# CasperTheCat/Vermilion

Measured on AMD Instinct MI355X. Metric: Mrays/sec (primary+secondary), 1920x1080 Sponza, higher is better.
Workload: dtype f32

## Files before the change

### vermilion_amd/csrc/api_render.inc

```
namespace {

Tuning make_tuning(const vmx_scene *sc, const vmx_opts *o) {
    Tuning tn;
    tn.refill_min = o->reserved[3] ? o->reserved[3] : 8u;
    tn.refill_primary = o->reserved[3] ? o->reserved[3] : 64u;
    tn.shade_min = o->reserved[4] ? o->reserved[4] : 16u;
    tn.leaf_min = 0xFFFFFFFFu;
    tn.sort_mode = o->reserved[5];
    tn.two_phase = false;
    tn.sorted = false;
    tn.bounce_records = false;
    tn.pool = false;
    tn.guide = false;
    const uint32_t cap = o->reserved[6];
    tn.lds_entries = std::min(sc->dev.stack_entries, cap ? cap : 10u);
    tn.lds_primary = std::min(sc->dev.stack_entries, cap ? cap : (uint32_t)VMX_LDS_PRIMARY);
    tn.lds_bounce = std::min(sc->dev.stack_entries, cap ? cap : 9u);
    tn.tail_threshold = o->reserved[2] ? o->reserved[2] : (16u << 20);
    return tn;
}


int bind_stack(vmx_scene *sc, const Tuning &tn, uint32_t entries, uint32_t grid, uint64_t items, WorkDev &wk, bool guided = false) {
    const uint64_t per_lane = items / ((uint64_t)grid * kPathsBlock);
// ... 368 lines not shown
        if (ws.full_mask.ensure(words + 8) || ws.full_u32.ensure(2 * words + 16) || ws.full_tmp.ensure(tmp + 256))
            return fail(VMX_ERR_NOMEM, "hipMalloc failed for the two-phase shading lists");
        ws.full_words = words, ws.full_tmp_bytes = tmp;
    }
    if (job.split_any && (tn.sorted || tn.bounce_records)) {
        const size_t waves = (size_t)sc->num_cus * ((size_t)std::max(job.tb, job.tbb) + (tn.guide ? kGuideFallbackBlocks : 0u)) * (kPathsBlock / 64);
        ws.out_capacity = (size_t)n_pad_max * smax + waves * 256 + 1024;
        if (ws.out_capacity > 0xFFFFFFFFull) return fail(VMX_ERR_INVALID, "pass too large for the sorted ray records");
        if (ws.out_rec.ensure(ws.out_capacity * (tn.sorted ? 32 : 16)) || ws.out_count.ensure(32))
            return fail(VMX_ERR_NOMEM, "hipMalloc failed for the ray records");
    }
    if (job.split_any) {
        if (ws.guide_ctr.ensure(2) || (tn.guide && (ws.guide_fb.ensure((size_t)job.qi[0].sub_capacity * kSubQueues) ||
                                                    ws.guide_fb_count.ensure(32) || ws.guide_heads.ensure(32))))
            return fail(VMX_ERR_NOMEM, "hipMalloc failed for the guide tree's fallback list");
    }
    if (job.elide) {
        if (ws.live_mask.ensure(job.live_words_max + 8) || ws.live_u32.ensure(2 * job.live_words_max + 16) ||
            ws.live_ids.ensure((size_t)n_pad_max * smax + 64) || ws.live_tmp.ensure(job.live_tmp_bytes + 256))
            return fail(VMX_ERR_NOMEM, "hipMalloc failed for the live-path list");
    }
    if (ws.rad.ensure((size_t)n_pad_max * smax * 16) || ws.next_count.ensure(32) || ws.counters.ensure(1) ||
        (tn.guide && ws.guide_fused_ctr.ensure(2)))
        return fail(VMX_ERR_NOMEM, "hipMalloc failed for the render workspace");
    job.px = PixelStateDev{job.pixels->accum.p, job.pixels->count.p, job.pixels->cursor.p};
    if (job.split_any) {
        const size_t n_inner = std::max<size_t>(sc->n_inner, 1);
        if (ws.cam_inner.ensure(n_inner * 64 * 8 + (size_t)sc->ntris * 64))
            return fail(VMX_ERR_NOMEM, "hipMalloc failed for the camera tables");
        LAUNCH_TRY(launch_camera_tables(sc->dev, sc->n_inner, fr.px, fr.py, fr.pz, ws.cam_inner.p,
                                        ws.cam_inner.p + n_inner * 64 * 8, s));
        job.launches++;
    }
    job.claims = job.claim_lists = nullptr;
    if (job.claims_on) {
        uint32_t expect = fr.early_stop ? std::min(fr.kmax, fr.nmin + 1 + (fr.quarter ? fr.kmax / fr.quarter - 1u : 0u)) : fr.kmax;
        if (run_samples) expect = std::min(expect, run_samples);
        if (expect >= claim_min_samples()) {
            int rc = timed_begin(ws, job.timed, s, -1, VMX_K_OTHER);
            if (rc) return rc;
            if ((rc = build_claims(sc, fr, tn, job.npix, job.lists_on, s))) return rc;
            if ((rc = timed_end(job.timed, s))) return rc;
            job.claims = ws.claims.p;
            if (job.lists_on) job.claim_lists = ws.claim_lists.p;
            job.launches++;
        }
    }
    if (job.claims && job.fuse_on) {
        const size_t words = n_pad_max / 64;
        const size_t tmp = live_compact_tmp_bytes((uint32_t)words);
        if (ws.unclaimed.ensure((size_t)n_pad_max + 64) || ws.claimed_slots.ensure((size_t)n_pad_max + 64) || ws.unclaimed_mask.ensure(words + 8) || ws.unclaimed_u32.ensure(2 * words + 16) ||
            ws.unclaimed_tmp.ensure(tmp + 256))
            return fail(VMX_ERR_NOMEM, "hipMalloc failed for the list of unclaimed pixels");
        ws.unclaimed_words = words, ws.unclaimed_tmp_bytes = tmp;
    }
    return VMX_OK;
}

int render_pass(vmx_scene *sc, RenderJob &job, uint32_t cap, uint32_t *taken) {
    Workspace &ws = sc->ws;
    FrameDev &fr = job.fr;
    const Tuning &tn = job.tn;
    const uint32_t pipeline = job.pipeline, smax = job.smax, n_active = job.n_active, n_pad_max = job.n_pad_max;
    const bool count = job.count, elide = job.elide;
    const int cur_list = job.cur_list;
    PixelStateDev px = job.px;
    PathArrays &pa = job.pa;
    IdQueue *qi = job.qi;
    hipStream_t s = job.s;
    std::vector<TimedLaunch> &timed = job.timed;
    uint64_t &launches = job.launches;
    unsigned int *act_cur = job.pixels->active[cur_list].p, *act_next = job.pixels->active[cur_list ^ 1].p;
    int rc;
    *taken = 0;
    uint32_t S;
    if (fr.early_stop) {
        fr.lead = 0;
        if (job.n_uniform < fr.nmin + 1 && job.n_uniform < fr.kmax) {
            S = std::min({fr.nmin + 1 - job.n_uniform, smax, fr.kmax - job.n_uniform, cap});
            job.n_uniform += S;
            const uint32_t strata_after = fr.quarter ? fr.kmax / fr.quarter - 1u : 0u;
            if (S == fr.nmin + 1 && S <= fr.quarter && strata_after > 0 && S + strata_after <= std::min(smax, cap)) {
                fr.lead = S;
                S += strata_after;
            }
        } else {
            constexpr uint64_t spec = 16ull << 20, spec_cap = 1024;
            S = std::max(1u, fr.kmax / std::max(fr.quarter, 1u) - 1u);
            if ((job.last_pass_pixels > 0 && job.last_pass_breaks * 8 < job.last_pass_pixels) || (uint64_t)n_active * 2 * spec_cap <= spec)
                S = (uint32_t)std::min<uint64_t>(std::max<uint64_t>(1, spec / (2ull * n_active)), spec_cap);
            S = (uint32_t)std::min<uint64_t>(S, ((uint64_t)n_pad_max * job.smax_alloc) / ((n_active + 63u) & ~63u));
            S = std::max(std::min(S, cap), 1u);
        }
    } else if (job.ragged) {
        S = std::min(smax, cap);
    } else {
        if (job.k_fixed >= fr.kmax) {
            job.n_active = 0;
            return VMX_OK;
        }
        S = std::min({smax, fr.kmax - job.k_fixed, cap});
        job.k_fixed += S;
    }
    *taken = S;
    const uint32_t n_pad = (n_active + 63u) & ~63u;
    const bool split = pipeline == 4 || (pipeline == 0 && (uint64_t)n_pad * S >= ((fr.early_stop && job.frame_passes > 0) ? kHybridLeftover : kHybridPaths));
    const bool refill = pipeline == 1 || (pipeline == 0 && !split);
    WorkDev wk;
    std::memset(&wk, 0, sizeof(wk));
    wk.heads = ws.heads.p;
    wk.nsrc = 8;
    wk.refill_min = split ? tn.refill_primary : tn.refill_min, wk.shade_min = tn.shade_min;
    wk.active = act_cur;
    wk.n_active = n_active, wk.n_pad = n_pad, wk.samples = S, wk.div_samples = make_fastdiv(S);
    wk.band_slots = (((n_pad + 7u) / 8u) + 63u) & ~63u;
    wk.band_items = wk.band_slots * S;
    wk.pixel_major = 1;
    if (split) {
        wk.cam_inner = ws.cam_inner.p, wk.cam_tris = ws.cam_inner.p + std::max<size_t>(sc->n_inner, 1) * 64 * 8;
        wk.cam_n_inner = sc->n_inner;
        wk.claims = job.claims;
        wk.claim_lists = elide ? nullptr : job.claim_lists, wk.list_ctr = ws.counters.p;
        const bool fuse = job.fuse_on && job.claims && (S & 63u) == 0;
        LaunchCfg cfg = paths_cfg(sc, tn.lds_primary, (uint64_t)n_pad * S, job.tb);
        rc = bind_stack(sc, tn, tn.lds_primary, cfg.grid, (uint64_t)n_pad * S, wk);
        if (rc) return rc;
        HIP_TRY(hipMemsetAsync(ws.heads.p, 0, kSubQueues * 32 * 4, s));
        if ((rc = timed_begin(ws, timed, s, -1, VMX_K_RAYGEN))) return rc;
        if (elide) {
            const uint32_t nwords = (uint32_t)(((uint64_t)n_pad * S + 63) / 64);
            unsigned int *cnt = ws.live_u32.p, *offs = cnt + job.live_words_max, *len = offs + job.live_words_max;
            wk.live_mask = ws.live_mask.p, wk.live_cnt = cnt;
            LAUNCH_TRY(launch_raygen(sc->dev, fr, wk, px, pa, s));
            HIP_TRY((hipError_t)launch_live_compact(ws.live_mask.p, cnt, nwords, offs, ws.live_ids.p, len, ws.live_tmp.p, job.live_tmp_bytes, s));
            wk.live_ids = ws.live_ids.p, wk.live_count = len;
            LAUNCH_TRY(launch_raygen_live(sc->dev, fr, wk, px, pa, s));
            HIP_TRY(hipMemsetAsync(pa.rad_mask, 0, (size_t)nwords * 8, s));
        } else {
            if (fuse) {
                const uint32_t nwords = n_pad / 64;
                unsigned int *cnt = ws.unclaimed_u32.p, *offs = cnt + ws.unclaimed_words, *len = offs + ws.unclaimed_words;
                LAUNCH_TRY(launch_unclaimed_words(act_cur, n_active, n_pad, job.claims, ws.unclaimed_mask.p, cnt, s));
                HIP_TRY((hipError_t)launch_slot_lists(ws.unclaimed_mask.p, cnt, nwords, n_active, offs, ws.unclaimed.p, ws.claimed_slots.p, len,
                                                      ws.unclaimed_tmp.p, ws.unclaimed_tmp_bytes, s));
                wk.unclaimed = ws.unclaimed.p, wk.unclaimed_count = len;
                launches += 3;
            }
            LAUNCH_TRY(launch_raygen(sc->dev, fr, wk, px, pa, s));
        }
        if (tn.sorted) {
            wk.out_rec = ws.out_rec.p, wk.out_count = ws.out_count.p, wk.out_ctr = ws.counters.p, wk.out_capacity = (uint32_t)ws.out_capacity;
            HIP_TRY(hipMemsetAsync(ws.out_count.p, 0, 4, s));
            if (!elide) HIP_TRY(hipMemsetAsync(pa.rad_mask, 0, (size_t)(((uint64_t)n_pad * S + 63) / 64) * 8, s));
        }
        if ((rc = timed_end(timed, s))) return rc;
        if ((rc = timed_begin(ws, timed, s, 0, VMX_K_TRACE_CAMERA))) return rc;
        {
            WorkDev wt = wk;
            if (fuse) wt.claims = nullptr;
            LAUNCH_TRY(launch_trace_q(sc->dev, fr, wt, px, pa, ws.counters.p, count, false, cfg, s));
        }
        if ((rc = timed_end(timed, s))) return rc;
        HIP_TRY(hipMemsetAsync(qi[0].counts, 0, kSubQueues * 32 * 4, s));
        if ((rc = timed_begin(ws, timed, s, 2, VMX_K_SHADE_CAMERA))) return rc;
        if (tn.two_phase && !elide && !tn.sorted) {
            if ((rc = shade_two_phase(sc, fr, wk, px, pa, qi, qi[0], 0, (size_t)(((uint64_t)n_pad * S + 63) / 64), false, ws.counters.p, false, s))) return rc;
        } else {
            if (fuse) {
                WorkDev wsh = wk;
                wsh.shade_slots = wk.unclaimed, wsh.shade_count = wk.unclaimed_count;
                LAUNCH_TRY(launch_shade(sc->dev, fr, wsh, px, pa, qi[0], 0, ws.counters.p, false, s));
                wsh.shade_slots = ws.claimed_slots.p, wsh.shade_count = wk.unclaimed_count + 1, wsh.fused = 1;
                LAUNCH_TRY(launch_shade(sc->dev, fr, wsh, px, pa, qi[0], 0, ws.counters.p, false, s));
                launches++;
            } else {
                LAUNCH_TRY(launch_shade(sc->dev, fr, wk, px, pa, qi[0], 0, ws.counters.p, false, s));
            }
        }
        if ((rc = timed_end(timed, s))) return rc;
        launches += 4;
        rc = run_ids(sc, fr, pa, qi, 0, ws.counters.p, count, tn, s, timed, launches, job.tbb, job.rb);
        if (rc) return rc;
    } else if (refill) {
        LaunchCfg cfg = paths_cfg(sc, tn.lds_entries, (uint64_t)n_pad * S, job.rb);
        rc = bind_stack(sc, tn, tn.lds_entries, cfg.grid, (uint64_t)n_pad * S, wk, tn.guide);
        if (rc) return rc;
        HIP_TRY(hipMemsetAsync(ws.heads.p, 0, kSubQueues * 32 * 4, s));
        if ((rc = timed_begin(ws, timed, s, 0, VMX_K_FUSED))) return rc;
        const GuidePathsDev gp = guide_paths(sc, tn);
        LAUNCH_TRY(launch_paths(sc->dev, fr, wk, px, ws.rad.p, ws.counters.p, count, cfg, s, &gp));
        if ((rc = timed_end(timed, s))) return rc;
        launches += 2;
    } else {
        rc = ab_legacy_pass(sc, job, act_cur, n_active, S);
        if (rc) return rc;
    }
    HIP_TRY(hipMemsetAsync(ws.next_count.p, 0, 8, s));
    if ((rc = timed_begin(ws, timed, s, -1, VMX_K_RESOLVE))) return rc;
    LAUNCH_TRY(launch_resolve(fr, act_cur, n_active, S, split || refill, ws.rad.p, split ? pa.rad_mask : nullptr, px, act_next,
                              ws.next_count.p, job.d_out, ws.counters.p, s, job.moments));
    if ((rc = timed_end(timed, s))) return rc;
    launches++;
    job.passes++;
    job.frame_passes++;
    unsigned int h_next[2] = {0, 0};
    HIP_TRY(hipMemcpyAsync(h_next, ws.next_count.p, 8, hipMemcpyDeviceToHost, s));
    HIP_TRY(hipStreamSynchronize(s));
    job.last_pass_pixels = n_active;
    job.last_pass_breaks = h_next[1];
    job.n_active = h_next[0];
    job.cur_list ^= 1;
    return VMX_OK;
// ... 436 lines not shown
```

### vermilion_amd/csrc/vmx_host.h

```cpp
namespace {

thread_local std::string g_err;

int fail(int code, const std::string &msg) {
    g_err = msg;
    return code;
}

#define HIP_TRY(expr)                                                                              \
    do {                                                                                           \
        hipError_t e_ = (expr);                                                                    \
        if (e_ != hipSuccess)                                                                      \
            return fail(VMX_ERR_HIP, std::string(#expr) + ": " + hipGetErrorString(e_));           \
    } while (0)

#define LAUNCH_TRY(expr)                                                                           \
    do {                                                                                           \
        int e_ = (expr);                                                                           \
        if (e_ != 0)                                                                               \
            return fail(VMX_ERR_HIP, std::string(#expr) + ": " + hipGetErrorString((hipError_t)e_)); \
    } while (0)

const vmx_sphere kReferenceSpheres[8] = {
    {{15.f, 140.f, 25.f}, 3.5f, {0.f * 15.f, .5f * 15.f, 1.0f * 15.f}, VMX_SPHERE_EMIT, {-55.f, 350.f, -150.f}, -1.f},
// ... 60 lines not shown
            hipEvent_t e;
            if (hipEventCreate(&e) != hipSuccess) return nullptr;
            ev.push_back(e);
        }
        return ev[used++];
    }
    void reset() { used = 0; }
};

struct Fence : NoCopy {
    hipEvent_t ev = nullptr;
    bool recorded = false;
    ~Fence() { if (ev) (void)hipEventDestroy(ev); }
    int wait(hipStream_t s) const {
        if (recorded) HIP_TRY(hipStreamWaitEvent(s, ev, 0));
        return VMX_OK;
    }
    int record(hipStream_t s) {
        if (!ev) HIP_TRY(hipEventCreateWithFlags(&ev, hipEventDisableTiming));
        HIP_TRY(hipEventRecord(ev, s));
        recorded = true;
        return VMX_OK;
    }
    int sync() const {
        if (recorded) HIP_TRY(hipEventSynchronize(ev));
        return VMX_OK;
    }
};

struct PixelBufs {
    DevBuf<unsigned char> accum;
    DevBuf<unsigned int> count, cursor, active[2];
    int ensure(size_t npix) {
        return accum.ensure(npix * 16) || count.ensure(npix) || cursor.ensure(npix) || active[0].ensure(npix) || active[1].ensure(npix);
    }
};

struct Workspace {
    DevBuf<unsigned char> queue_planes[2];
    DevBuf<unsigned int> queue_counts;
    DevBuf<unsigned int> heads;
    DevBuf<unsigned char> overflow_stack;
    DevBuf<unsigned char> rayA, state, hit, thr;
    DevBuf<unsigned int> ids[3], id_counts;
    DevBuf<unsigned int> sort_keys[2], ids_sorted;
    DevBuf<unsigned char> sort_tmp;
    DevBuf<unsigned char> cam_inner;
    DevBuf<unsigned int> claims;
    DevBuf<unsigned int> claim_lists;
    DevBuf<unsigned int> unclaimed, claimed_slots, unclaimed_u32;
    DevBuf<unsigned long long> unclaimed_mask;
    DevBuf<unsigned char> unclaimed_tmp;
    size_t unclaimed_words = 0, unclaimed_tmp_bytes = 0;
    DevBuf<unsigned char> rad;
    DevBuf<unsigned long long> rad_mask;
    DevBuf<unsigned long long> live_mask;
    DevBuf<unsigned int> live_u32, live_ids;
    DevBuf<unsigned char> live_tmp;
    DevBuf<unsigned long long> full_mask;
    DevBuf<unsigned int> full_u32;
    DevBuf<unsigned char> full_tmp;
    size_t full_words = 0, full_tmp_bytes = 0;
    DevBuf<unsigned char> out_rec;
    DevBuf<unsigned int> out_count;
    size_t out_capacity = 0;
    DevBuf<unsigned int> guide_fb, guide_fb_count, guide_heads;
    DevBuf<unsigned long long> guide_ctr;
    DevBuf<unsigned long long> guide_fused_ctr;
    uint64_t guide_entries = 0;
    PixelBufs pixels;
    DevBuf<unsigned int> next_count;
    DevBuf<DevCounters> counters;
    DevBuf<float> out;
    std::vector<unsigned int> order;
    uint32_t order_w = 0, order_rows = 0;
    EventPool events;
};

}

#define VMX_OPAQUE __attribute__((visibility("hidden")))

struct vmx_scene {
    int device = 0;
    int num_cus = 0;
    DevStream stream;
    HostBvh bvh;
    LbvhDevice lbvh;
    bool device_built = false;
    uint32_t builder = VMX_BVH_REFERENCE;
    std::atomic<bool> flat_ready{true};
    bool flat_topology = true;
    uint32_t n_inner = 0;
    uint32_t ntris = 0, leaf_size = 4;
    std::vector<vmx_sphere> spheres;
    DevBuf<unsigned char> d_geom;
    DevBuf<AttrRecord> d_attrs;
    DevBuf<SphereDev> d_spheres;
    DevBuf<float> d_tex, d_tex1;
    uint32_t n_textures = 0;
    SceneDev dev{};
    std::mutex mu;
    Workspace ws;
    uint32_t block = 256;
    float bounds_lo[3] = {0, 0, 0}, bounds_hi[3] = {1, 1, 1};
    vmx_timings timings{};
// ... 236 lines not shown
```

### vermilion_amd/csrc/vmx_kernels.h

```cpp
#pragma once
#include <stdint.h>
#include "vmx_device.h"

namespace vmx {

constexpr uint32_t kSubQueues = 16;

struct QueueDev {
    void *planes;
    unsigned int *counts;
    uint32_t capacity;
    uint32_t sub_capacity;
};

struct PixelStateDev {
    void *accum;
    unsigned int *count;
    unsigned int *cursor;
};

struct PathArrays {
    void *rayA;
    void *state;
    void *hit;
// ... 98 lines not shown
                   LaunchCfg cfg, void *stream);
int launch_primary_ids(const SceneDev &sc, const FrameDev &fr, uint32_t k, int32_t *tri_id, float *t,
                       LaunchCfg cfg, void *stream);

constexpr uint32_t kQueryCastRays = 3, kQueryCastCamera = 4, kQueryModes = 5;
int launch_query(const SceneDev &sc, const QueryDev &q, uint32_t mode, bool quad, LaunchCfg cfg, void *stream);
int query_query_blocks_per_cu(uint32_t block, uint32_t lds_bytes, uint32_t mode, bool quad, int *blocks);
int launch_raycast_query(const SceneDev &sc, const QueryDev &q, const FrameDev &fr, bool camera, bool quad, void *out,
                         LaunchCfg cfg, uint32_t finish_grid, void *stream);

struct RefitItem {
    uint32_t ref, dst;
};
constexpr uint32_t kRefitRoot = 0xFFFFFFFFu;
int launch_update_records(uint32_t ntris, const float *pos, const float *nrm, const float *uv, void *tris, void *attrs,
                          void *stream);
int launch_refit_level(const RefitItem *items, uint32_t n, const float *pos, const void *tris, void *inner,
                       float *root_box, void *stream);
int launch_attrs_by_id(uint32_t ntris, const void *tris, const void *attrs, float *nrm, float *uv, void *stream);

int launch_trig(const float *x, uint32_t n, float *cs, float *sn, void *stream);

int launch_init_pixels(PixelStateDev px, uint32_t npix, void *stream);
int launch_zero_u32(unsigned int *p, uint32_t n, void *stream);
#ifdef VMX_AB_KERNELS
int launch_primary(const SceneDev &sc, const FrameDev &fr, const unsigned int *active,
                   uint32_t n_active, uint32_t samples, PixelStateDev px, QueueDev qout, void *rad,
                   DevCounters *counters, bool count, bool loop_to_end, LaunchCfg cfg, void *stream);
int launch_radiance_init(const float *o, const float *d, uint32_t n, uint64_t seed, QueueDev qout,
                         void *stream);
int launch_bounce(const SceneDev &sc, float r2scale, uint32_t libm_double, QueueDev qin, uint32_t max_chunks, QueueDev qout,
                  void *rad, DevCounters *counters, bool count, bool loop_to_end, bool first_step,
                  LaunchCfg cfg, void *stream);
int query_blocks_per_cu(uint32_t block, uint32_t lds_bytes, bool count, int *primary_blocks, int *bounce_blocks);
int launch_trace_pool(const SceneDev &sc, const WorkDev &wk, PathArrays pa, LaunchCfg cfg, void *stream);
int query_trace_pool(uint32_t block, uint32_t pool_slots, uint32_t lds_levels, uint32_t *lds_bytes, int *blocks);
#endif
int launch_paths(const SceneDev &sc, const FrameDev &fr, const WorkDev &wk, PixelStateDev px, void *rad,
                 DevCounters *counters, bool count, LaunchCfg cfg, void *stream, const GuidePathsDev *guide = nullptr);
int query_paths_blocks_per_cu(uint32_t block, uint32_t lds_bytes, bool count, int *blocks, bool guide = false);
int launch_camera_tables(const SceneDev &sc, uint32_t n_inner, float ox, float oy, float oz, void *cam_inner,
                         void *cam_tris, void *stream);
int launch_pixel_claims(const SceneDev &sc, const FrameDev &fr, const WorkDev &wk, unsigned int *claims, unsigned int *lists, unsigned int *n_claimed,
                        LaunchCfg cfg, void *stream);
int launch_raygen(const SceneDev &sc, const FrameDev &fr, const WorkDev &wk, PixelStateDev px, PathArrays pa, void *stream);
int launch_raygen_live(const SceneDev &sc, const FrameDev &fr, const WorkDev &wk, PixelStateDev px, PathArrays pa, void *stream);
size_t live_compact_tmp_bytes(uint32_t nwords);
int launch_live_compact(const unsigned long long *live_mask, const unsigned int *live_cnt, uint32_t nwords,
                        unsigned int *offs, unsigned int *ids, unsigned int *count, void *tmp, size_t tmp_bytes, void *stream);
int launch_slot_lists(const unsigned long long *mask, const unsigned int *cnt, uint32_t nwords, uint32_t n_active, unsigned int *offs,
                      unsigned int *unclaimed, unsigned int *claimed, unsigned int *counts, void *tmp, size_t tmp_bytes, void *stream);
int launch_unclaimed_words(const unsigned int *active, uint32_t n_active, uint32_t n_pad, const unsigned int *claims,
                           unsigned long long *mask, unsigned int *cnt, void *stream);
int launch_trace_q(const SceneDev &sc, const FrameDev &fr, const WorkDev &wk, PixelStateDev px, PathArrays pa,
                   DevCounters *counters, bool count, bool from_queue, LaunchCfg cfg, void *stream, const GuideDev *guide = nullptr,
                   unsigned int *visits = nullptr);
int query_trace_q_blocks_per_cu(uint32_t block, uint32_t lds_bytes, bool count, bool from_queue, bool sorted, bool live, int *blocks,
                                bool guide = false);
int launch_shade(const SceneDev &sc, const FrameDev &fr, const WorkDev &wk, PixelStateDev px, PathArrays pa,
                 IdQueue qout, uint32_t max_chunks, DevCounters *counters, bool from_queue, void *stream);
int launch_shade_ends(const SceneDev &sc, const FrameDev &fr, const WorkDev &wk, PathArrays pa, unsigned long long *full_mask,
                      unsigned int *full_cnt, uint32_t max_chunks, DevCounters *counters, bool from_queue, void *stream);
int launch_tail(const SceneDev &sc, const FrameDev &fr, const WorkDev &wk, PathArrays pa, DevCounters *counters,
                bool count, LaunchCfg cfg, void *stream, const GuidePathsDev *guide = nullptr);
int launch_radiance_init_ids(const float *o, const float *d, uint32_t n, uint64_t seed, PathArrays pa,
                             IdQueue qout, void *stream);
int launch_resolve(const FrameDev &fr, const unsigned int *active, uint32_t n_active, uint32_t samples,
                   bool pixel_major, const void *rad, const unsigned long long *rad_mask, PixelStateDev px, unsigned int *next_active,
                   unsigned int *next_count, float *out_rgbaz, DevCounters *counters, void *stream, bool moments = false);
int launch_list_words(const unsigned int *list, uint32_t n, const unsigned char *select, const unsigned int *cursor, uint32_t kmax,
                      unsigned long long *mask, unsigned int *cnt, void *stream);
int launch_list_compact(const unsigned long long *mask, const unsigned int *cnt, uint32_t nwords, unsigned int *offs,
                        const unsigned int *src, unsigned int *dst, unsigned int *count, void *tmp, size_t tmp_bytes, void *stream);
struct SamplingPass {
    uint32_t width, height;
    uint32_t kmax, min_samples, radius;
    float threshold, floor;
    PixelStateDev px;
};
int launch_sampling_error(const SamplingPass &a, float *error, float *variance, void *stream);
int launch_sampling_select(const SamplingPass &a, unsigned char *select, unsigned int *count, void *stream);
int launch_bruteforce(const SceneDev &sc, const FrameDev &fr, const unsigned int *order, uint32_t npix, uint32_t flags,
                      float *out, DevCounters *counters, void *longs , unsigned int *long_count,
                      const WorkDev &stack , LaunchCfg cfg, void *stream);
int launch_bruteforce_long(const SceneDev &sc, const FrameDev &fr, uint32_t flags, float *out, DevCounters *counters,
                           const void *longs, const unsigned int *long_count, uint32_t count, const WorkDev &stack,
                           LaunchCfg cfg, void *stream);
int launch_preview(PixelStateDev px, uint32_t npix, uint32_t kmax, const float *finished, float *out_rgbaz, void *rgba8,
                   void *stream);
struct FilterSrc {
    const float *frame;
    PixelStateDev px;
    const float *finished;
    uint32_t kmax;
};
struct FilterPass {
    uint32_t width, height;
    uint32_t step;
    uint32_t squarings;
    float isc2, kz;
    const void *guide;
    FilterSrc src;
    const void *in_plane;
    void *out_plane;
    float *out_rgbaz;
    void *rgba8;
// ... 91 lines not shown
```

### vermilion_amd/csrc/vmx_kernels.hip

```cpp
#include <hip/hip_runtime.h>
#include <math.h>
#include <algorithm>
#include <stdint.h>

#include "vmx_kernels.h"
#include "pixel_claim.h"
#include "guide_walk.h"
#include <type_traits>

#ifndef VMX_CAM_BATCH
#define VMX_CAM_BATCH 16
#endif
#ifndef VMX_TRACE_WAVES_PER_SIMD
#define VMX_TRACE_WAVES_PER_SIMD 7
#endif


namespace vmx {
__device__ __forceinline__ float luminance(float r, float g, float b);
namespace {

constexpr float kInf = __builtin_huge_valf();

struct Cnt {
// ... 1446 lines not shown
    __device__ __forceinline__ void put(int i, uint32_t ref, float near) { stack_push(stk, ovf, lds_entries, i, make_uint2(ref, __float_as_uint(near))); }
    __device__ __forceinline__ void get(int i, uint32_t &ref, float &near) const {
        const uint2 e = stack_pop(stk, ovf, lds_entries, i);
        ref = e.x, near = __uint_as_float(e.y);
    }
};
__global__ void __launch_bounds__(256)
k_pixel_claims(SceneDev sc, FrameDev fr, const float *__restrict__ cam_inner, const float *__restrict__ cam_tris,
               unsigned int *__restrict__ claims, unsigned int *__restrict__ lists, unsigned int *n_claimed, uint32_t lds_levels,
               uint32_t overflow_entries, void *overflow_stack) {
    extern __shared__ uint2 lds_stack[];
    const uint32_t lane = threadIdx.x & 63u, wave = threadIdx.x >> 6;
    ClaimStack stk;
    stk.stk = lds_stack + (size_t)wave * (lds_levels + 1) * 64 + lane;
    stk.ovf = (uint2 *)overflow_stack + ((size_t)(blockIdx.x * (blockDim.x >> 6) + wave) * overflow_entries) * 64 + lane;
    stk.lds_entries = (int)lds_levels;
    PcFilm fm;
    for (int i = 0; i < 9; ++i) fm.m[i] = fr.m[i];
    fm.width = fr.width, fm.height = fr.height, fm.sensor_x = fr.sensor_x, fm.sensor_y = fr.sensor_y, fm.film_dist = fr.film_dist;
    const uint32_t tiles_x = (fr.width + 7u) / 8u, tiles = tiles_x * ((fr.local_rows + 7u) / 8u);
    uint32_t n = 0;
    for (uint32_t tile = blockIdx.x * (blockDim.x >> 6) + wave; tile < tiles; tile += gridDim.x * (blockDim.x >> 6)) {
        const uint32_t ty = tile / tiles_x, tx = tile - ty * tiles_x;
        const uint32_t x = tx * 8u + (lane & 7u), y = ty * 8u + (lane >> 3);
        if (x < fr.width && y < fr.local_rows) {
            const uint32_t lp = y * fr.width + x;
            uint32_t c;
            if (lists) {
                uint32_t l[kListWords];
                c = pc_pixel_claim_and_list(fm, global_pixel(fr, lp), cam_inner, cam_tris, sc.root_ref, stk,
                                            (int)(lds_levels + overflow_entries), l);
                ((uint4 *)lists)[lp] = make_uint4(l[0], l[1], l[2], l[3]);
            } else {
                c = pc_pixel_claim(fm, global_pixel(fr, lp), cam_inner, cam_tris, sc.root_ref, stk, (int)(lds_levels + overflow_entries));
            }
            claims[lp] = c;
            n += c != kClaimNone ? 1u : 0u;
        }
    }
    n = wave_sum(n);
    if (lane == 0 && n) atomicAdd(n_claimed, n);
}

__global__ void __launch_bounds__(256)
k_unclaimed_words(const unsigned int *__restrict__ active, uint32_t n_active, uint32_t n_pad, const unsigned int *__restrict__ claims,
                  unsigned long long *__restrict__ mask, unsigned int *__restrict__ cnt) {
    for (uint32_t s_idx = blockIdx.x * blockDim.x + threadIdx.x; s_idx < n_pad; s_idx += gridDim.x * blockDim.x) {
        const bool un = s_idx < n_active && claims[active[s_idx]] == kClaimNone;
        const unsigned long long bits = __builtin_amdgcn_ballot_w64(un);
        if ((threadIdx.x & 63u) == 0) mask[s_idx >> 6] = bits, cnt[s_idx >> 6] = (uint32_t)__popcll(bits);
    }
}

template <int LIVE>
__global__ void __launch_bounds__(256)
k_raygen(SceneDev sc, FrameDev fr, WorkDev wk, PixelStateDev px, PathArrays pa) {
    const uint32_t total = wk.samples * wk.n_pad;
    if (wk.pixel_major && (wk.samples & 63u) == 0) {
        const uint32_t lane = threadIdx.x & 63u;
        const uint32_t waves = gridDim.x * (blockDim.x >> 6);
        const uint32_t chunks = wk.samples >> 6;
        const bool listed = !LIVE && wk.unclaimed != nullptr;
        const uint32_t units = listed ? *wk.unclaimed_count : wk.n_pad;
        for (uint32_t unit = (uint32_t)__builtin_amdgcn_readfirstlane((int)(blockIdx.x * (blockDim.x >> 6) + (threadIdx.x >> 6)));
             unit < units; unit += waves) {
            const uint32_t s_idx = listed ? wk.unclaimed[unit] : unit;
            const uint32_t pid_base = s_idx * wk.samples;
            if (s_idx < wk.n_active) {
                const uint32_t lp = wk.active[s_idx];
                const uint32_t pixel = global_pixel(fr, lp);
                const PixelKey pk = rng_pixel_key(fr.seed, pixel);
                const bool lights = (LIVE || fr.camera_bits) && pixel_may_reach_a_light(sc, fr, pixel);
                const uint32_t cur = px.cursor[lp];
                const uint32_t k0 = cur & ~kCursorStrided, kstep = (cur & kCursorStrided) ? fr.quarter : 1u;
                for (uint32_t ch = 0; ch < chunks; ++ch) {
                    const uint32_t j = ch * 64u + lane;
                    const uint32_t k = (fr.lead != 0 && j >= fr.lead) ? (j - fr.lead + 1u) * fr.quarter : k0 + j * kstep;
                    bool live = false;
                    float dx = 0.f, dy = 0.f, dz = 0.f;
                    uint32_t depth = 0xFFFFFFFFu;
                    if (k < fr.kmax) {
                        Rng rng;
                        if (LIVE && !lights) {
                            rng_init_keyed(rng, pk, k);
                            (void)rng_next(rng);
                            (void)rng_next(rng);
                            live = step_bits<false>(sc, fr.r2scale, rng, 0, fr.px, fr.py, fr.pz, 0.f, 0.f, 0.f, 1.f, 1.f, 1.f, false) != 3u;
                        } else {
                            primary_ray_keyed(fr, pixel, pk, k, rng, dx, dy, dz);
                            if (LIVE) live = !step_is_dead<false>(sc, fr.r2scale, rng, 0, fr.px, fr.py, fr.pz, dx, dy, dz, 1.f, 1.f, 1.f);
                            else depth = fr.camera_bits ? step_bits<false>(sc, fr.r2scale, rng, 0, fr.px, fr.py, fr.pz, dx, dy, dz, 1.f, 1.f, 1.f, lights) : 0u;
                        }
                    }
                    if (!LIVE) ((float4 *)pa.rayA)[pid_base + j] = make_float4(dx, dy, dz, __uint_as_float(depth));
                    if (LIVE) {
                        const unsigned long long bits = __builtin_amdgcn_ballot_w64(live);
                        if (lane == 0) wk.live_mask[(pid_base >> 6) + ch] = bits, wk.live_cnt[(pid_base >> 6) + ch] = (uint32_t)__popcll(bits);
                    }
                }
            } else {
                for (uint32_t ch = 0; ch < chunks; ++ch) {
                    if (!LIVE) ((float4 *)pa.rayA)[pid_base + ch * 64u + lane] = make_float4(0.f, 0.f, 0.f, __uint_as_float(0xFFFFFFFFu));
                    if (LIVE && lane == 0) wk.live_mask[(pid_base >> 6) + ch] = 0ull, wk.live_cnt[(pid_base >> 6) + ch] = 0u;
                }
            }
        }
        return;
    }
    for (uint32_t pid = blockIdx.x * blockDim.x + threadIdx.x; pid < total; pid += gridDim.x * blockDim.x) {
        uint32_t j, s_idx;
        if (wk.pixel_major) s_idx = fast_div(pid, wk.div_samples), j = pid - s_idx * wk.samples;
        else j = pid / wk.n_pad, s_idx = pid - j * wk.n_pad;
        uint32_t pid2, pixel, k;
        float dx = 0.f, dy = 0.f, dz = 0.f;
        uint32_t depth = 0xFFFFFFFFu;
        bool live = false;
        if (s_idx < wk.n_active && primary_item(fr, wk, px, j, s_idx, pid2, pixel, k)) {
            Rng rng;
            primary_ray(fr, pixel, k, rng, dx, dy, dz);
            if (LIVE) live = !step_is_dead<false>(sc, fr.r2scale, rng, 0, fr.px, fr.py, fr.pz, dx, dy, dz, 1.f, 1.f, 1.f);
            else depth = fr.camera_bits ? step_bits<false>(sc, fr.r2scale, rng, 0, fr.px, fr.py, fr.pz, dx, dy, dz, 1.f, 1.f, 1.f) : 0u;
        }
        if (!LIVE) ((float4 *)pa.rayA)[pid] = make_float4(dx, dy, dz, __uint_as_float(depth));
        if (LIVE) {
            const unsigned long long bits = __builtin_amdgcn_ballot_w64(live);
            if ((threadIdx.x & 63u) == 0) wk.live_mask[pid >> 6] = bits, wk.live_cnt[pid >> 6] = (uint32_t)__popcll(bits);
        }
    }
}

__global__ void __launch_bounds__(256)
k_raygen_live(SceneDev sc, FrameDev fr, WorkDev wk, PixelStateDev px, PathArrays pa) {
    const uint32_t n = *wk.live_count;
    for (uint32_t i = blockIdx.x * blockDim.x + threadIdx.x; i < n; i += gridDim.x * blockDim.x) {
        const uint32_t pid = wk.live_ids[i];
        uint32_t j, s_idx;
        if (wk.pixel_major) s_idx = fast_div(pid, wk.div_samples), j = pid - s_idx * wk.samples;
        else j = pid / wk.n_pad, s_idx = pid - j * wk.n_pad;
        uint32_t pid2, pixel, k;
        float dx = 0.f, dy = 0.f, dz = 0.f;
        uint32_t depth = 0xFFFFFFFFu;
        if (primary_item(fr, wk, px, j, s_idx, pid2, pixel, k)) {
            Rng rng;
            primary_ray(fr, pixel, k, rng, dx, dy, dz);
            depth = fr.camera_bits ? step_bits<false>(sc, fr.r2scale, rng, 0, fr.px, fr.py, fr.pz, dx, dy, dz, 1.f, 1.f, 1.f) : 0u;
        }
        ((float4 *)pa.rayA)[i] = make_float4(dx, dy, dz, __uint_as_float(depth));
    }
}

__device__ __forceinline__ uint32_t live_band(uint32_t n) { return ((n + 511u) / 512u) * 64u; }

template <bool COUNT, int SRC>
__global__ void __launch_bounds__(256, VMX_TRACE_WAVES_PER_SIMD)
k_trace_q(SceneDev sc, FrameDev fr, WorkDev wk, PixelStateDev px, PathArrays pa, DevCounters *ctr) {
    extern __shared__ uint2 lds_stack[];
    const uint32_t lane = threadIdx.x & 63u, wave = threadIdx.x >> 6;
    const int lds_entries = (int)wk.lds_entries;
// ... 1208 lines not shown
#define VMX_GO(C, T) \
    hipLaunchKernelGGL((k_paths<C, 0, T>), g, b, cfg.lds_bytes, s, sc, fr, wk, px, (float4 *)rad, pa, counters)
    PathArrays pa{};
    if (guide && guide->off && !count) {
        if (sc.tex) hipLaunchKernelGGL((k_paths<false, 0, true, GuidePathsDev>), g, b, cfg.lds_bytes, s, sc, fr, wk, px, (float4 *)rad, pa, counters, *guide);
        else hipLaunchKernelGGL((k_paths<false, 0, false, GuidePathsDev>), g, b, cfg.lds_bytes, s, sc, fr, wk, px, (float4 *)rad, pa, counters, *guide);
    } else if (sc.tex) {
        if (count) VMX_GO(true, true);
        else VMX_GO(false, true);
    } else {
        if (count) VMX_GO(true, false);
        else VMX_GO(false, false);
    }
#undef VMX_GO
    return launch_status();
}

int launch_tail(const SceneDev &sc, const FrameDev &fr, const WorkDev &wk, PathArrays pa, DevCounters *counters,
                bool count, LaunchCfg cfg, void *stream, const GuidePathsDev *guide) {
    hipStream_t s = (hipStream_t)stream;
    dim3 g(cfg.grid), b(cfg.block);
    PixelStateDev px{nullptr, nullptr, nullptr};
#define VMX_GO(C, T) \
    hipLaunchKernelGGL((k_paths<C, 2, T>), g, b, cfg.lds_bytes, s, sc, fr, wk, px, (float4 *)pa.rad, pa, counters)
    if (guide && guide->off && !count) {
        if (sc.tex) hipLaunchKernelGGL((k_paths<false, 2, true, GuidePathsDev>), g, b, cfg.lds_bytes, s, sc, fr, wk, px, (float4 *)pa.rad, pa, counters, *guide);
        else hipLaunchKernelGGL((k_paths<false, 2, false, GuidePathsDev>), g, b, cfg.lds_bytes, s, sc, fr, wk, px, (float4 *)pa.rad, pa, counters, *guide);
    } else if (sc.tex) {
        if (count) VMX_GO(true, true);
        else VMX_GO(false, true);
    } else {
        if (count) VMX_GO(true, false);
        else VMX_GO(false, false);
    }
#undef VMX_GO
    return launch_status();
}

int launch_camera_tables(const SceneDev &sc, uint32_t n_inner, float ox, float oy, float oz, void *cam_inner,
                         void *cam_tris, void *stream) {
    const uint32_t total = n_inner + sc.ntris;
    uint32_t grid = std::min<uint32_t>((total + 255) / 256, 4096);
    if (grid == 0) grid = 1;
    hipLaunchKernelGGL(k_camera_tables, dim3(grid), dim3(256), 0, (hipStream_t)stream, sc, n_inner, ox, oy, oz,
                       (float4 *)cam_inner, (float4 *)cam_tris);
    return launch_status();
}

int launch_raygen(const SceneDev &sc, const FrameDev &fr, const WorkDev &wk, PixelStateDev px, PathArrays pa, void *stream) {
    const uint64_t total = (uint64_t)wk.samples * wk.n_pad;
    uint32_t grid = (uint32_t)std::min<uint64_t>((total + 255) / 256, 256u * 32u);
    if (grid == 0) grid = 1;
    if (wk.live_mask) hipLaunchKernelGGL(k_raygen<1>, dim3(grid), dim3(256), 0, (hipStream_t)stream, sc, fr, wk, px, pa);
    else hipLaunchKernelGGL(k_raygen<0>, dim3(grid), dim3(256), 0, (hipStream_t)stream, sc, fr, wk, px, pa);
    return launch_status();
}

int launch_pixel_claims(const SceneDev &sc, const FrameDev &fr, const WorkDev &wk, unsigned int *claims, unsigned int *lists, unsigned int *n_claimed,
                        LaunchCfg cfg, void *stream) {
    hipLaunchKernelGGL(k_pixel_claims, dim3(cfg.grid), dim3(cfg.block), cfg.lds_bytes, (hipStream_t)stream, sc, fr,
                       (const float *)wk.cam_inner, (const float *)wk.cam_tris, claims, lists, n_claimed, wk.lds_entries, wk.overflow_entries,
                       wk.overflow_stack);
    return launch_status();
}

int launch_unclaimed_words(const unsigned int *active, uint32_t n_active, uint32_t n_pad, const unsigned int *claims,
                           unsigned long long *mask, unsigned int *cnt, void *stream) {
    const uint32_t grid = std::max(1u, std::min<uint32_t>((n_pad + 255) / 256, 4096u));
    hipLaunchKernelGGL(k_unclaimed_words, dim3(grid), dim3(256), 0, (hipStream_t)stream, active, n_active, n_pad, claims, mask, cnt);
    return launch_status();
}

int launch_raygen_live(const SceneDev &sc, const FrameDev &fr, const WorkDev &wk, PixelStateDev px, PathArrays pa, void *stream) {
    const uint64_t total = ((uint64_t)wk.samples * wk.n_pad + 2) / 3;
    uint32_t grid = (uint32_t)std::min<uint64_t>((total + 255) / 256, 256u * 32u);
    if (grid == 0) grid = 1;
    hipLaunchKernelGGL(k_raygen_live, dim3(grid), dim3(256), 0, (hipStream_t)stream, sc, fr, wk, px, pa);
    return launch_status();
}

using TraceWKernel = void (*)(SceneDev, FrameDev, WorkDev, PathArrays, GuideDev);
using TraceQKernel = void (*)(SceneDev, FrameDev, WorkDev, PixelStateDev, PathArrays, DevCounters *);
static TraceWKernel trace_w_kernel(bool from_queue, bool sorted, bool live, bool guide) {
    if (from_queue) {
        if (guide) {
            if (sorted) return k_trace_w<1, false, true, true>;
            return k_trace_w<1, false, false, true>;
        }
        if (sorted) return k_trace_w<1, false, true>;
        return k_trace_w<1>;
    }
    if (sorted) {
        if (live) return k_trace_w<0, true, true>;
        return k_trace_w<0, false, true>;
    }
    if (live) return k_trace_w<0, true>;
    return k_trace_w<0>;
}
static TraceQKernel trace_q_kernel(bool from_queue) {
    if (from_queue) return k_trace_q<true, 1>;
    return k_trace_q<true, 0>;
}

int launch_trace_q(const SceneDev &sc, const FrameDev &fr, const WorkDev &wk, PixelStateDev px, PathArrays pa,
                   DevCounters *counters, bool count, bool from_queue, LaunchCfg cfg, void *stream, const GuideDev *guide,
                   unsigned int *visits) {
    hipStream_t s = (hipStream_t)stream;
// ... 181 lines not shown
```

### vermilion_amd/csrc/vmx_trace_w.inc

```
#if VMX_TRACE_W_VISITS
__global__ void __launch_bounds__(256, VMX_TRACE_WAVES_PER_SIMD) __attribute__((amdgpu_num_sgpr(VMX_TRACE_SGPRS)))
k_trace_w_visits(SceneDev sc, FrameDev fr, WorkDev wk, PathArrays pa, GuideDev gd, uint2 *visits_out) {
    constexpr int SRC = 1;
    constexpr bool LIVE = false, SORT = false, GUIDE = true, VISITS = true;
#else
template <int SRC, bool LIVE = false, bool SORT = false, bool GUIDE = false>
__global__ void __launch_bounds__(256, VMX_TRACE_WAVES_PER_SIMD) __attribute__((amdgpu_num_sgpr(VMX_TRACE_SGPRS)))
k_trace_w(SceneDev sc, FrameDev fr, WorkDev wk, PathArrays pa, GuideDev gd) {
    constexpr bool VISITS = false;
#endif
    static_assert(!GUIDE || (SRC == 1 && !LIVE), "the guide is for bounce rays");
    static_assert(!VISITS || GUIDE, "visits are counted on the guide walk");
    [[maybe_unused]] uint32_t n_inner = 0, n_tris = 0;
    extern __shared__ uint2 lds_stack[];
    const uint32_t lane = threadIdx.x & 63u, wave = threadIdx.x >> 6;
    const int lds_entries = (int)wk.lds_entries;
#ifdef VMX_STEP_PROFILE
    __shared__ unsigned long long s_prof[4][10][2];
    if (lane < 20) s_prof[wave][lane >> 1][lane & 1] = 0;
    unsigned long long prof_t = __builtin_readcyclecounter();
    if (lane == 0) atomicMin(&g_wave_span[SRC][0], (unsigned long long)wall_clock64());
#endif
    uint2 *stk = lds_stack + (size_t)wave * (lds_entries + 1) * 64 + lane;
    uint2 *ovf = (uint2 *)wk.overflow_stack +
// ... 149 lines not shown
                        tf1 = vmin3(r2.y * ix, r2.z * iy, r2.w * iz);
                    } else {
                        box_net(r0.x * ix, r0.y * iy, r0.z * iz, r0.w * ix, r1.x * iy, r1.y * iz, tn0, tf0);
                        box_net(r1.z * ix, r1.w * iy, r2.x * iz, r2.y * ix, r2.z * iy, r2.w * iz, tn1, tf1);
                    }
                    lref = __float_as_uint(r3.x), rref = __float_as_uint(r3.y);
                } else {
                    const float4 *rec = (const float4 *)((const char *)inner + (uint32_t)(cur << 6));
                    const float4 q0 = rec[0], q1 = rec[1], q2 = rec[2];
                    const float2 q3 = *(const float2 *)(rec + 3);
                    child_boxes_rel<EXACT>(q0, q1, q2, ix, iy, iz, tn0, tf0, tn1, tf1);
                    lref = __float_as_uint(q3.x), rref = __float_as_uint(q3.y);
                }
                cur = choose_child_masks(tn0, tf0, tn1, tf1, lref, rref, best, push);
            } else if ((int)cur < 0) {
                const uint32_t ti = (cur & kLeafStartMask) * 4;
                const float4 a = tris[ti], b = tris[ti + 1], c = tris[ti + 2];
                const float cd = ((const float *)tris)[ti * 4 + 12];
                float dist;
                const bool hit = tri_test_cam(a, b, c, cd, dx, dy, dz, dist);
                if (hit && dist < best) {
                    best = dist;
                    slot = (int)(cur & kLeafStartMask);
                }
                cur = leaf_advance(cur);
            }
        }
        if (cur == kPop) {
            cur = pop_to_next(stk, ovf, lds_entries, sp, GUIDE ? cut : best);
            if (cur == kBottom) {
#if VMX_TRACE_W_VISITS
                visits_out[pid] = make_uint2(n_inner, n_tris);
#endif
                if (SORT || GUIDE) rflags |= 0x80000000u;
                else hit_out[pid] = make_float2(best, __int_as_float(slot));
                cur = kIdle;
            }
        }
    };

    for (;;) {
        const unsigned long long idle = __builtin_amdgcn_ballot_w64(cur == kIdle);
        if (idle != 0 && !exhausted && ((uint32_t)__popcll(idle) >= refill_min || idle == ~0ull)) {
            if (GUIDE) guide_finished();
            if (SORT) sort_finished();
            for (;;) {
                if (res_lo == res_hi) {
                    uint32_t lim = SRC == 0 ? band_items : min(wk.qids.counts[src * 32], wk.qids.sub_capacity);
                    if (LIVE) {
                        const uint32_t n = *wk.live_count, seg = live_band(n);
                        lim = min(seg, n - min(n, src * seg));
                    }
                    if (SRC == 0 && !LIVE && !SORT && wk.unclaimed) {
                        const uint32_t n = *wk.unclaimed_count, seg = (n + nsrc - 1u) / nsrc;
                        lim = min(seg, n - min(n, src * seg)) * wk.samples;
                    }
                    uint32_t base = 0;
                    if (lane == 0) base = atomicAdd(&wk.heads[src * 32], kReserve);
                    base = __builtin_amdgcn_readfirstlane(base);
                    if (base >= lim) {
                        src = (src + 1 == nsrc) ? 0 : src + 1;
                        if (++tried == nsrc) {
                            exhausted = true;
                            break;
                        }
                        continue;
                    }
                    tried = 0;
                    res_lo = base;
                    res_hi = min(base + kReserve, lim);
                }
                const unsigned long long want = __builtin_amdgcn_ballot_w64(cur == kIdle);
                if (want == 0) break;
                const uint32_t avail = res_hi - res_lo;
                const uint32_t rank = (uint32_t)__popcll(want & lt_mask);
                const bool take = cur == kIdle && rank < avail;
                const uint32_t item = res_lo + rank;
                res_lo = __builtin_amdgcn_readfirstlane(res_lo + min((uint32_t)__popcll(want), avail));
                bool listed = false;
                bool unwalked = false;
                if (take) {
                    bool valid = true;
                    uint32_t claim = kClaimNone;
                    uint4 lrec = make_uint4(kClaimNone, kClaimNone, kClaimNone, kClaimNone);
                    if (LIVE) {
                        pid = src * live_band(*wk.live_count) + item;
                    } else if (SRC == 0) {
                        uint32_t j, s_idx;
                        if (!SORT && wk.unclaimed) {
                            const uint32_t sl = fast_div(item, wk.div_samples), n = *wk.unclaimed_count;
                            j = item - sl * wk.samples, s_idx = wk.unclaimed[src * ((n + nsrc - 1u) / nsrc) + sl];
                        } else if (wk.pixel_major) {
                            const uint32_t sl = fast_div(item, wk.div_samples);
                            j = item - sl * wk.samples, s_idx = src * band_slots + sl;
                        } else {
                            j = item / band_slots, s_idx = src * band_slots + (item - j * band_slots);
                        }
                        valid = s_idx < wk.n_active;
                        pid = path_id(wk, j, s_idx);
                        if (wk.claims && valid) claim = wk.claims[wk.active[s_idx]];
                        if (wk.claim_lists && valid && claim == kClaimNone) lrec = ((const uint4 *)wk.claim_lists)[wk.active[s_idx]];
                    } else {
                        pid = wk.qids.ids[(size_t)src * wk.qids.sub_capacity + item];
                    }
                    if (valid) {
                        if (SRC == 0) {
                            const float4 a = ((const float4 *)pa.rayA)[pid];
                            ox = fr.px, oy = fr.py, oz = fr.pz, dx = a.x, dy = a.y, dz = a.z;
                            valid = __float_as_uint(a.w) != 0xFFFFFFFFu;
                            if (SORT && valid) rflags = __float_as_uint(a.w) & 7u;
                        } else {
                            const float4 a = ((const float4 *)pa.state)[(size_t)pid * 4], b = ((const float4 *)pa.state)[(size_t)pid * 4 + 1];
                            ox = a.x, oy = a.y, oz = a.z, dx = a.w, dy = b.x, dz = b.y;
                            valid = __float_as_uint(b.z) != 0xFFFFFFFFu;
                            if (SORT && valid) rflags = __float_as_uint(b.w) & 7u;
                        }
                    }
                    if (SRC == 0 && !LIVE && valid && claim != kClaimNone) {
                        best = 999999999.f, slot = -1;
                        if (claim != kClaimMiss) {
                            const float4 a = tris[claim * 4], b = tris[claim * 4 + 1], c = tris[claim * 4 + 2];
                            const float cd = ((const float *)tris)[claim * 16 + 12];
                            float dist;
                            if (tri_test_cam(a, b, c, cd, dx, dy, dz, dist) && dist < best) best = dist, slot = (int)claim;
                        }
                        if (SORT) rflags |= 0x80000000u;
                        else hit_out[pid] = make_float2(best, __int_as_float(slot));
                        valid = false;
                    }
                    if (SRC == 0 && !LIVE && valid && lrec.x != kClaimNone) {
                        float t;
                        uint32_t m;
                        if (pc_list_settle((const float *)tris, lrec.x, lrec.y, lrec.z, lrec.w, dx, dy, dz, t, m)) {
                            best = t, slot = (int)m;
                            if (SORT) rflags |= 0x80000000u;
                            else hit_out[pid] = make_float2(best, __int_as_float(slot));
                            valid = false, listed = true;
                        }
                    }
                    if (valid) {
                        ray_start(dx, dy, dz, root_ref, 999999999.f, ix, iy, iz, best, slot, sp, cur);
                        exact = !(finite3(ix, iy, iz) && finite3(ox, oy, oz));
                        if (GUIDE) {
                            cut = best * kGwCut, second = 3.0e38f;
                            exact = false;
                            if (VISITS) n_inner = n_tris = 0;
                            if (!gw_ray_ok(ox, oy, oz, dx, dy, dz, ix, iy, iz, gd.scene_max)) cur = kIdle, unwalked = true;
                        }
                    }
                }
                if (GUIDE) fallback_append(unwalked);
                if (SRC == 0 && !LIVE && wk.claim_lists) n_listed += (uint32_t)__popcll(__builtin_amdgcn_ballot_w64(listed));
                if (SRC == 0 && !LIVE && SORT && wk.claims) {
                    if (__builtin_amdgcn_ballot_w64((rflags >> 31) != 0) != 0) sort_finished();
// ... 95 lines not shown
```

Before: 12360.

## Settle claim-list camera rays in raygen and trace only walk pixels plus stragglers

Camera rays whose pixels carry a claim list are now resolved inside raygen with a small triangle-list test. Hits are written directly and only failures go into a straggler queue. The camera trace then walks just the pixels with neither a claim nor a list, through a new compacted walk-slot list, plus the stragglers as an extra source band. This aims to remove redundant BVH-walk setup and divergence for list pixels in the trace kernel. In exchange it adds a mask and compaction pass, atomics in raygen, and a possible overflow path if the straggler queue fills.

```diff
diff --git a/vermilion_amd/csrc/api_render.inc b/vermilion_amd/csrc/api_render.inc
--- a/vermilion_amd/csrc/api_render.inc
+++ b/vermilion_amd/csrc/api_render.inc
@@ -444,6 +444,8 @@
         if (ws.unclaimed.ensure((size_t)n_pad_max + 64) || ws.claimed_slots.ensure((size_t)n_pad_max + 64) || ws.unclaimed_mask.ensure(words + 8) || ws.unclaimed_u32.ensure(2 * words + 16) ||
             ws.unclaimed_tmp.ensure(tmp + 256))
             return fail(VMX_ERR_NOMEM, "hipMalloc failed for the list of unclaimed pixels");
+        if (job.claim_lists && (ws.walk_slots.ensure((size_t)n_pad_max + 64) || ws.walk_mask.ensure(words + 8) || ws.walk_u32.ensure(2 * words + 16)))
+            return fail(VMX_ERR_NOMEM, "hipMalloc failed for the list of walk slots");
         ws.unclaimed_words = words, ws.unclaimed_tmp_bytes = tmp;
     }
     return VMX_OK;
@@ -514,6 +516,9 @@
         wk.claims = job.claims;
         wk.claim_lists = elide ? nullptr : job.claim_lists, wk.list_ctr = ws.counters.p;
         const bool fuse = job.fuse_on && job.claims && (S & 63u) == 0;
+        const bool rays_settle_lists = fuse && !elide && wk.claim_lists != nullptr;
+        unsigned int *walk_len = nullptr;
+        IdQueue stragglers{};
         LaunchCfg cfg = paths_cfg(sc, tn.lds_primary, (uint64_t)n_pad * S, job.tb);
         rc = bind_stack(sc, tn, tn.lds_primary, cfg.grid, (uint64_t)n_pad * S, wk);
         if (rc) return rc;
@@ -538,7 +543,21 @@
                 wk.unclaimed = ws.unclaimed.p, wk.unclaimed_count = len;
                 launches += 3;
             }
-            LAUNCH_TRY(launch_raygen(sc->dev, fr, wk, px, pa, s));
+            WorkDev wr = wk;
+            if (rays_settle_lists) {
+                const uint32_t nwords = n_pad / 64;
+                unsigned int *cnt = ws.walk_u32.p, *offs = cnt + ws.unclaimed_words;
+                walk_len = offs + ws.unclaimed_words;
+                LAUNCH_TRY(launch_walk_words(act_cur, n_active, n_pad, job.claims, job.claim_lists, ws.walk_mask.p, cnt, s));
+                HIP_TRY((hipError_t)launch_live_compact(ws.walk_mask.p, cnt, nwords, offs, ws.walk_slots.p, walk_len, ws.unclaimed_tmp.p,
+                                                        ws.unclaimed_tmp_bytes, s));
+                HIP_TRY(hipMemsetAsync(qi[2].counts, 0, 4, s));
+                wr.qids.ids = qi[2].ids, wr.qids.counts = qi[2].counts;
+                wr.qids.sub_capacity = (uint32_t)std::min<uint64_t>((uint64_t)qi[2].sub_capacity * kSubQueues, 0xFFFFFFFFull);
+                launches += 2;
+            }
+            LAUNCH_TRY(launch_raygen(sc->dev, fr, wr, px, pa, s));
+            if (rays_settle_lists) stragglers = wr.qids;
         }
         if (tn.sorted) {
             wk.out_rec = ws.out_rec.p, wk.out_count = ws.out_count.p, wk.out_ctr = ws.counters.p, wk.out_capacity = (uint32_t)ws.out_capacity;
@@ -550,6 +569,10 @@
         {
             WorkDev wt = wk;
             if (fuse) wt.claims = nullptr;
+            if (rays_settle_lists) {
+                wt.unclaimed = ws.walk_slots.p, wt.unclaimed_count = walk_len, wt.claim_lists = nullptr;
+                wt.qids = stragglers, wt.nsrc = 9;
+            }
             LAUNCH_TRY(launch_trace_q(sc->dev, fr, wt, px, pa, ws.counters.p, count, false, cfg, s));
         }
         if ((rc = timed_end(timed, s))) return rc;
diff --git a/vermilion_amd/csrc/vmx_host.h b/vermilion_amd/csrc/vmx_host.h
--- a/vermilion_amd/csrc/vmx_host.h
+++ b/vermilion_amd/csrc/vmx_host.h
@@ -136,6 +136,8 @@
     DevBuf<unsigned long long> unclaimed_mask;
     DevBuf<unsigned char> unclaimed_tmp;
     size_t unclaimed_words = 0, unclaimed_tmp_bytes = 0;
+    DevBuf<unsigned int> walk_slots, walk_u32;
+    DevBuf<unsigned long long> walk_mask;
     DevBuf<unsigned char> rad;
     DevBuf<unsigned long long> rad_mask;
     DevBuf<unsigned long long> live_mask;
diff --git a/vermilion_amd/csrc/vmx_kernels.h b/vermilion_amd/csrc/vmx_kernels.h
--- a/vermilion_amd/csrc/vmx_kernels.h
+++ b/vermilion_amd/csrc/vmx_kernels.h
@@ -174,6 +174,8 @@
                       unsigned int *unclaimed, unsigned int *claimed, unsigned int *counts, void *tmp, size_t tmp_bytes, void *stream);
 int launch_unclaimed_words(const unsigned int *active, uint32_t n_active, uint32_t n_pad, const unsigned int *claims,
                            unsigned long long *mask, unsigned int *cnt, void *stream);
+int launch_walk_words(const unsigned int *active, uint32_t n_active, uint32_t n_pad, const unsigned int *claims,
+                      const unsigned int *lists, unsigned long long *mask, unsigned int *cnt, void *stream);
 int launch_trace_q(const SceneDev &sc, const FrameDev &fr, const WorkDev &wk, PixelStateDev px, PathArrays pa,
                    DevCounters *counters, bool count, bool from_queue, LaunchCfg cfg, void *stream, const GuideDev *guide = nullptr,
                    unsigned int *visits = nullptr);
diff --git a/vermilion_amd/csrc/vmx_kernels.hip b/vermilion_amd/csrc/vmx_kernels.hip
--- a/vermilion_amd/csrc/vmx_kernels.hip
+++ b/vermilion_amd/csrc/vmx_kernels.hip
@@ -1522,10 +1522,26 @@
     }
 }
 
-template <int LIVE>
+__global__ void __launch_bounds__(256)
+k_walk_words(const unsigned int *__restrict__ active, uint32_t n_active, uint32_t n_pad, const unsigned int *__restrict__ claims,
+             const unsigned int *__restrict__ lists, unsigned long long *__restrict__ mask, unsigned int *__restrict__ cnt) {
+    for (uint32_t s_idx = blockIdx.x * blockDim.x + threadIdx.x; s_idx < n_pad; s_idx += gridDim.x * blockDim.x) {
+        bool walk = false;
+        if (s_idx < n_active) {
+            const uint32_t lp = active[s_idx];
+            walk = claims[lp] == kClaimNone && lists[(size_t)lp * kListWords] == kClaimNone;
+        }
+        const unsigned long long bits = __builtin_amdgcn_ballot_w64(walk);
+        if ((threadIdx.x & 63u) == 0) mask[s_idx >> 6] = bits, cnt[s_idx >> 6] = (uint32_t)__popcll(bits);
+    }
+}
+
+template <int LIVE, bool LISTS = false>
 __global__ void __launch_bounds__(256)
 k_raygen(SceneDev sc, FrameDev fr, WorkDev wk, PixelStateDev px, PathArrays pa) {
+    static_assert(!LISTS || !LIVE, "list pixels are settled in the plain form");
     const uint32_t total = wk.samples * wk.n_pad;
+    [[maybe_unused]] uint32_t n_listed = 0;
     if (wk.pixel_major && (wk.samples & 63u) == 0) {
         const uint32_t lane = threadIdx.x & 63u;
         const uint32_t waves = gridDim.x * (blockDim.x >> 6);
@@ -1543,6 +1559,9 @@
                 const bool lights = (LIVE || fr.camera_bits) && pixel_may_reach_a_light(sc, fr, pixel);
                 const uint32_t cur = px.cursor[lp];
                 const uint32_t k0 = cur & ~kCursorStrided, kstep = (cur & kCursorStrided) ? fr.quarter : 1u;
+                typedef uint32_t u32x4 __attribute__((ext_vector_type(4)));
+                [[maybe_unused]] u32x4 lrec = {kClaimNone, kClaimNone, kClaimNone, kClaimNone};
+                if constexpr (LISTS) lrec = ((const __attribute__((address_space(4))) u32x4 *)(uintptr_t)wk.claim_lists)[lp];
                 for (uint32_t ch = 0; ch < chunks; ++ch) {
                     const uint32_t j = ch * 64u + lane;
                     const uint32_t k = (fr.lead != 0 && j >= fr.lead) ? (j - fr.lead + 1u) * fr.quarter : k0 + j * kstep;
@@ -1567,6 +1586,27 @@
                         const unsigned long long bits = __builtin_amdgcn_ballot_w64(live);
                         if (lane == 0) wk.live_mask[(pid_base >> 6) + ch] = bits, wk.live_cnt[(pid_base >> 6) + ch] = (uint32_t)__popcll(bits);
                     }
+                    if constexpr (LISTS) {
+                        if (lrec.x != kClaimNone) {
+                            const float *ctris = (const float *)(const __attribute__((address_space(4))) float *)(uintptr_t)wk.cam_tris;
+                            const bool has = depth != 0xFFFFFFFFu;
+                            float t = 0.f;
+                            uint32_t m = 0;
+                            const bool settled = has && pc_list_settle(ctris, lrec.x, lrec.y, lrec.z, lrec.w, dx, dy, dz, t, m);
+                            if (settled) ((float2 *)pa.hit)[pid_base + j] = make_float2(t, __int_as_float((int)m));
+                            n_listed += (uint32_t)__popcll(__builtin_amdgcn_ballot_w64(settled));
+                            const bool strag = has && !settled;
+                            const unsigned long long sm = __builtin_amdgcn_ballot_w64(strag);
+                            if (sm != 0) {
+                                uint32_t base = 0;
+                                if (lane == 0) base = atomicAdd(wk.qids.counts, (uint32_t)__popcll(sm));
+                                base = __builtin_amdgcn_readfirstlane(base);
+                                const uint32_t at = base + (uint32_t)__popcll(sm & ((1ull << lane) - 1ull));
+                                if (strag && at < wk.qids.sub_capacity) wk.qids.ids[at] = pid_base + j;
+                                else if (strag) atomicAdd(&wk.list_ctr->overflow, 1ull);
+                            }
+                        }
+                    }
                 }
             } else {
                 for (uint32_t ch = 0; ch < chunks; ++ch) {
@@ -1574,6 +1614,9 @@
                     if (LIVE && lane == 0) wk.live_mask[(pid_base >> 6) + ch] = 0ull, wk.live_cnt[(pid_base >> 6) + ch] = 0u;
                 }
             }
+        }
+        if constexpr (LISTS) {
+            if (lane == 0 && n_listed) atomicAdd(&wk.list_ctr->listed, (unsigned long long)n_listed);
         }
         return;
     }
@@ -2888,7 +2931,17 @@
     uint32_t grid = (uint32_t)std::min<uint64_t>((total + 255) / 256, 256u * 32u);
     if (grid == 0) grid = 1;
     if (wk.live_mask) hipLaunchKernelGGL(k_raygen<1>, dim3(grid), dim3(256), 0, (hipStream_t)stream, sc, fr, wk, px, pa);
-    else hipLaunchKernelGGL(k_raygen<0>, dim3(grid), dim3(256), 0, (hipStream_t)stream, sc, fr, wk, px, pa);
+    else if (wk.unclaimed && wk.claim_lists && wk.qids.ids) {
+        if (!wk.pixel_major || (wk.samples & 63u) != 0 || !wk.cam_tris || !wk.list_ctr || !wk.qids.counts) return (int)hipErrorInvalidValue;
+        hipLaunchKernelGGL((k_raygen<0, true>), dim3(grid), dim3(256), 0, (hipStream_t)stream, sc, fr, wk, px, pa);
+    } else hipLaunchKernelGGL(k_raygen<0>, dim3(grid), dim3(256), 0, (hipStream_t)stream, sc, fr, wk, px, pa);
+    return launch_status();
+}
+
+int launch_walk_words(const unsigned int *active, uint32_t n_active, uint32_t n_pad, const unsigned int *claims,
+                      const unsigned int *lists, unsigned long long *mask, unsigned int *cnt, void *stream) {
+    const uint32_t grid = std::max(1u, std::min<uint32_t>((n_pad + 255) / 256, 4096u));
+    hipLaunchKernelGGL(k_walk_words, dim3(grid), dim3(256), 0, (hipStream_t)stream, active, n_active, n_pad, claims, lists, mask, cnt);
     return launch_status();
 }
 
diff --git a/vermilion_amd/csrc/vmx_trace_w.inc b/vermilion_amd/csrc/vmx_trace_w.inc
--- a/vermilion_amd/csrc/vmx_trace_w.inc
+++ b/vermilion_amd/csrc/vmx_trace_w.inc
@@ -225,8 +225,9 @@
                         lim = min(seg, n - min(n, src * seg));
                     }
                     if (SRC == 0 && !LIVE && !SORT && wk.unclaimed) {
-                        const uint32_t n = *wk.unclaimed_count, seg = (n + nsrc - 1u) / nsrc;
-                        lim = min(seg, n - min(n, src * seg)) * wk.samples;
+                        const uint32_t nband = wk.qids.ids ? nsrc - 1u : nsrc;
+                        const uint32_t n = *wk.unclaimed_count, seg = (n + nband - 1u) / nband;
+                        lim = src == nband ? min(wk.qids.counts[0], wk.qids.sub_capacity) : min(seg, n - min(n, src * seg)) * wk.samples;
                     }
                     uint32_t base = 0;
                     if (lane == 0) base = atomicAdd(&wk.heads[src * 32], kReserve);
@@ -260,19 +261,29 @@
                         pid = src * live_band(*wk.live_count) + item;
                     } else if (SRC == 0) {
                         uint32_t j, s_idx;
+                        bool straggler = false;
                         if (!SORT && wk.unclaimed) {
-                            const uint32_t sl = fast_div(item, wk.div_samples), n = *wk.unclaimed_count;
-                            j = item - sl * wk.samples, s_idx = wk.unclaimed[src * ((n + nsrc - 1u) / nsrc) + sl];
+                            const uint32_t nband = wk.qids.ids ? nsrc - 1u : nsrc;
+                            if (src == nband) {
+                                straggler = true, j = 0, s_idx = 0;
+                            } else {
+                                const uint32_t sl = fast_div(item, wk.div_samples), n = *wk.unclaimed_count;
+                                j = item - sl * wk.samples, s_idx = wk.unclaimed[src * ((n + nband - 1u) / nband) + sl];
+                            }
                         } else if (wk.pixel_major) {
                             const uint32_t sl = fast_div(item, wk.div_samples);
                             j = item - sl * wk.samples, s_idx = src * band_slots + sl;
                         } else {
                             j = item / band_slots, s_idx = src * band_slots + (item - j * band_slots);
                         }
-                        valid = s_idx < wk.n_active;
-                        pid = path_id(wk, j, s_idx);
-                        if (wk.claims && valid) claim = wk.claims[wk.active[s_idx]];
-                        if (wk.claim_lists && valid && claim == kClaimNone) lrec = ((const uint4 *)wk.claim_lists)[wk.active[s_idx]];
+                        if (!SORT && straggler) {
+                            pid = wk.qids.ids[item];
+                        } else {
+                            valid = s_idx < wk.n_active;
+                            pid = path_id(wk, j, s_idx);
+                            if (wk.claims && valid) claim = wk.claims[wk.active[s_idx]];
+                            if (wk.claim_lists && valid && claim == kClaimNone) lrec = ((const uint4 *)wk.claim_lists)[wk.active[s_idx]];
+                        }
                     } else {
                         pid = wk.qids.ids[(size_t)src * wk.qids.sub_capacity + item];
                     }
```

After: 13030, median of 6. 5.4% higher.
